# blackle/Megalania

Hardware: AMD Instinct MI355X
Metric: SA neighbour-cost evals/s (higher is better)
Workload: dtype u64

## Files before the change

### megalania_amd/csrc/mgl_api.hip

```cpp
#include "mgl_kernels.hip"
#include "mgl_kernels2.hip"
#include "mgl_kernels3.hip"
#include "mgl_kernels4.hip"
#include "mgl_kernels5.hip"
#include "mgl_pbuild.hip"
#include "mgl_index.hip"
#include "mgl_matchfinder.hip"
#include "mgl_optimal.hip"
#include "mgl_adaptive.hip"
#include "mgl_props.hip"
#include "mgl_crossover.hip"
#include "../../include/megalania_hip.h"

#include <math.h>
#include <stdio.h>
#include <stdlib.h>
#include <string.h>
#include <string>
#include <vector>

static const uint16_t k_cost_table[2048] = {
#include "mgl_cost_table.inc"
};

// ... 65 lines not shown
	uint16_t* d_cost_tbl;
	BaseMem base, scratch;
	mgl_pk* d_best;
	NbrOut nbr;
	uint32_t* d_aos;
	uint64_t* d_cum;
	uint16_t* d_final_probs;
	mgl_pk* d_topk_pk;
	uint64_t* d_topk_cost;
	uint32_t* d_small;
	uint32_t* d_sub_offs;
	uint32_t* d_sub_lens;
	uint32_t sub_cap;
	uint64_t sqrt_thresh;
	uint32_t per_wave_bytes, waves_per_block, nbr_lds, walk_lds;
	bool incremental;
	Base2 b2;
	unsigned long long* d_prof;
	uint32_t* d_todo;
	uint32_t per_wave2, waves_per_block2, nbr2_lds, build_lds;
	uint32_t big_waves = MGL_BIG_WAVES;
	uint32_t chg_cap = MGL_CHG_CAP;
	uint32_t per_wave_pick, per_wave_rest, pick_waves;
	size_t b2_bytes;
	BigScratch big;
	uint32_t* d_todo2;
	uint4* d_pickstate;
	uint4* d_pickrec;
	bool split_nbr, adaptive;
	bool form_single = false;
	uint32_t* d_counts;
	ApplyBuf ab;
	uint32_t apply_blocks;
	bool incremental_apply;
	bool snapshots;
	Base2 snap_lit, snap_best;
	SnapMeta* d_snap_meta;
	bool parallel_build;
	PBuild pb;
	hipEvent_t ev_begin, ev_end;
	std::vector<hipEvent_t> ev_pool;
	int accept_mode = MGL_ACCEPT_AUTO;
	uint32_t bulk_threshold = 0;
	bool bulk_now = true;
	uint64_t bulk_hold = 0;
	uint64_t blk_done = 0;
// ... 286 lines not shown
	}
	if (!sa->incremental) {
		const uint32_t blocks = (K + sa->waves_per_block - 1) / sa->waves_per_block;
		hipLaunchKernelGGL(k_neighbours, dim3(blocks), dim3(64 * sa->waves_per_block), sa->nbr_lds, sa->stream, sa->ctx, sa->base.v,
		                   (const Control*)sa->base.ctl, sa->cfg.seed, step_override, K, sa->nbr, sa->per_wave_bytes,
		                   (const uint32_t*)nullptr, (const uint32_t*)nullptr); NBR_TRACE("k_neighbours");
		HIPCHK(hipGetLastError());
		return MGL_OK;
	}
	if (zero_counts) HIPCHK(hipMemsetAsync(sa->d_counts, 0, 8 * sizeof(uint32_t), sa->stream));
	const uint32_t blocks2 = (K + sa->waves_per_block2 - 1) / sa->waves_per_block2;
	const bool split_now = sa->split_nbr && !sa->form_single;
	const uint32_t sim_lds_regular = ((((sa->ctx.L.total + 31u) >> 5) + 3u) & ~3u) * 4u + sa->chg_cap * 16u;
	if (split_now) {
		const uint32_t slices = nbr_slices(sa);
		HIPCHK(hipEventRecord(sa->ev_fork, sa->stream));
		if (slices >= 2) HIPCHK(hipStreamWaitEvent(sa->stream2, sa->ev_fork, 0));
#if !MGL_TAIL_EARLY
		HIPCHK(hipStreamWaitEvent(sa->stream3, sa->ev_fork, 0));
#endif
		for (uint32_t h = 0; h < slices; h++) {
			const uint32_t j0 = (uint32_t)((uint64_t)K * h / slices), j1 = (uint32_t)((uint64_t)K * (h + 1) / slices);
			hipStream_t st = (h & 1u) ? sa->stream2 : sa->stream;
			hipLaunchKernelGGL((sa->d_prof ? k_neighbours2<false, MGL_NBR_PICK, true> : k_neighbours2<false, MGL_NBR_PICK>), dim3((j1 - j0 + sa->pick_waves - 1) / sa->pick_waves), dim3(64 * sa->pick_waves),
			                   (MGL_PICK_T_GLOBAL ? 0u : 4096u) + sa->pick_waves * sa->per_wave_pick, st, sa->ctx,
			                   sa->b2, sa->base.ctl, sa->cfg.seed, step_override, K, sa->nbr, sa->per_wave_pick, sa->d_todo, sa->d_counts,
			                   sa->d_prof, sa->big, sa->d_pickrec, j0, j1, sa->d_pickstate); NBR_TRACE("k_neighbours2<false, MGL_NBR_PICK>");
			hipLaunchKernelGGL((k_neighbours2<false, MGL_NBR_REST>), dim3(j1 - j0), dim3(64), sa->per_wave_rest, st, sa->ctx,
			                   sa->b2, sa->base.ctl, sa->cfg.seed, step_override, K, sa->nbr, sa->per_wave_rest, sa->d_todo, sa->d_counts,
			                   g_prof_big ? (unsigned long long*)nullptr : sa->d_prof, sa->big, sa->d_pickrec, j0, j1, sa->d_pickstate); NBR_TRACE("k_neighbours2<false, MGL_NBR_REST>");
			HIPCHK(hipEventRecord(sa->ev_rest[h], st));
		}
		HIPCHK(hipGetLastError());
		for (uint32_t h = 0; h < slices; h++) {
			const uint32_t j0 = (uint32_t)((uint64_t)K * h / slices), j1 = (uint32_t)((uint64_t)K * (h + 1) / slices);
			HIPCHK(hipStreamWaitEvent(sa->stream3, sa->ev_rest[h], 0));
			if (sa->time_sim_step >= 0 && h < 2) HIPCHK(hipEventRecord(sim_event(sa, 4 * (size_t)sa->time_sim_step + 2 * h), sa->stream3));
			if (sa->count_traffic)
				hipLaunchKernelGGL(k_sim<true>, dim3(j1 - j0), dim3(64 * sa->sim_waves), sim_lds_regular, sa->stream3, sa->ctx, sa->b2, sa->base.ctl,
				                   sa->nbr, sa->big, j0, j1, sa->d_traffic);
			else
				hipLaunchKernelGGL(k_sim<false>, dim3(j1 - j0), dim3(64 * sa->sim_waves), sim_lds_regular, sa->stream3, sa->ctx, sa->b2, sa->base.ctl,
				                   sa->nbr, sa->big, j0, j1, (unsigned long long*)nullptr);
			NBR_TRACE("k_sim");
			if (sa->time_sim_step >= 0 && h < 2) HIPCHK(hipEventRecord(sim_event(sa, 4 * (size_t)sa->time_sim_step + 2 * h + 1), sa->stream3));
		}
// ... 416 lines not shown
			HIPCHK(hipMemset(sa->d_todo2, 0, sizeof(uint32_t) * (K + 1)));
		}
		{
			uint32_t best_w = 1, best_total = 0;
			for (uint32_t w = 1; w <= 8; w++) {
				const uint32_t bytes = 4096u + w * sa->per_wave2;
				if (bytes > 160u * 1024u) break;
				const uint32_t tot = (160u * 1024u / bytes) * w;
				if (tot > best_total) { best_total = tot; best_w = w; }
			}
			(void)best_w;
			sa->waves_per_block2 = 1;
		}
		sa->nbr2_lds = 4096u + sa->waves_per_block2 * sa->per_wave2;
		sa->build_lds = 4096u + ckpt_elems * 2u + ckpt_elems * 8u;
		HIPCHK(hipMalloc(&sa->d_counts, sizeof(uint32_t) * 16));
		HIPCHK(hipMemset(sa->d_counts, 0, sizeof(uint32_t) * 16));
		sa->big.todo_in = sa->d_todo; sa->big.todo_in_count = sa->d_counts; sa->big.spill_ctr = sa->d_counts + 2;
		HIPCHK(hipFuncSetAttribute((const void*)k_neighbours2<false, MGL_NBR_FULL>, hipFuncAttributeMaxDynamicSharedMemorySize, (int)sa->nbr2_lds));
		HIPCHK(hipFuncSetAttribute((const void*)k_neighbours2<false, MGL_NBR_PICK>, hipFuncAttributeMaxDynamicSharedMemorySize, 160 * 1024));
		HIPCHK(hipFuncSetAttribute((const void*)k_neighbours2<false, MGL_NBR_PICK, true>, hipFuncAttributeMaxDynamicSharedMemorySize, 160 * 1024));
		HIPCHK(hipFuncSetAttribute((const void*)k_neighbours2<false, MGL_NBR_REST>, hipFuncAttributeMaxDynamicSharedMemorySize, (int)sa->nbr2_lds));
		HIPCHK(hipFuncSetAttribute((const void*)k_neighbours2<true, MGL_NBR_FULL>, hipFuncAttributeMaxDynamicSharedMemorySize, (int)(4096u + sa->per_wave2 + 12u * MGL_BIG_CAP + MGL_COOP_BYTES)));
		HIPCHK(hipMalloc(&sa->d_pickrec, sizeof(uint4) * K));
		HIPCHK(hipMalloc(&sa->d_pickstate, sizeof(uint4) * 2 * K));
		sa->split_nbr = getenv("MGL_NO_SPLIT") == nullptr;
		if (sa->split_nbr) {
			BigScratch& g = sa->big;
			HIPCHK(hipMalloc(&g.sim_hdr, sizeof(uint4) * (size_t)K));
			HIPCHK(hipMalloc(&g.sim_keys, sizeof(uint16_t) * 2u * sa->chg_cap * (size_t)K));
			HIPCHK(hipMalloc(&g.sim_pos, sizeof(uint32_t) * 2u * sa->chg_cap * (size_t)K));
			HIPCHK(hipMemset(g.sim_hdr, 0xFF, sizeof(uint4) * (size_t)K));
			if (getenv("MGL_NO_CONT") == nullptr) {
				HIPCHK(hipMalloc(&g.cont, sizeof(uint32_t) * MGL_CONT_WORDS * (size_t)g.slots));
				HIPCHK(hipMemset(g.cont, 0, sizeof(uint32_t) * MGL_CONT_WORDS * (size_t)g.slots));
			}
		}
		if (getenv("MGL_SIMW")) { const int w = atoi(getenv("MGL_SIMW")); if (w == 1 || w == 2 || w == 4 || w == 8) sa->sim_waves = (uint32_t)w; }
		sa->adaptive = sa->split_nbr && getenv("MGL_NO_ADAPT") == nullptr;
		sa->form_single = !sa->split_nbr;
		sa->pick_waves = getenv("MGL_PICK_WAVES") ? (uint32_t)atoi(getenv("MGL_PICK_WAVES")) : 0u;
		if (sa->pick_waves != 1 && sa->pick_waves != 2 && sa->pick_waves != 4 && sa->pick_waves != 8) sa->pick_waves = 0;
		{
			uint32_t best_w = 1, best_resident = 0;
			for (uint32_t w = 1; w <= 8; w *= 2) {
				const uint32_t bytes = (MGL_PICK_T_GLOBAL ? 0u : 4096u) + w * sa->per_wave_pick;
// ... 1351 lines not shown
		HIPCHK(hipMemcpy(v + 8, sa->d_counts, sizeof(uint32_t) * 8, hipMemcpyDeviceToHost));
		memcpy(out, v, sizeof v);
		return MGL_OK;
	}
	case 14: src = sa->ab.hdr; sz = sa->ab.hdr ? sizeof(uint32_t) * 16 : 0; break;
	case 16: src = sa->base.ctl; sz = sizeof(Control); break;
	case 15: src = sa->d_pickrec; sz = sa->d_pickrec ? sizeof(uint4) * sa->cfg.neighbours_per_step : 0; break;
	case 18: src = sa->d_quad_pos; sz = sizeof(uint32_t) * (sa->n - 1); break;
	case 19: src = sa->d_quad_nx; sz = sizeof(uint16_t) * (sa->n - 1); break;
	case 12: src = sa->d_bucket_off; sz = sizeof(uint32_t) * 65537; break;
	case 13: src = sa->d_bucket_pos; sz = sizeof(uint32_t) * (sa->n - 1); break;
	case 30: case 31: case 32: case 33: case 34: case 35: src = sa->d_xpos[what - 30]; sz = sizeof(uint32_t) * (sa->n - 1); break;
	case 40: case 41: case 42: case 43: case 44: case 45: src = sa->d_xrank[what - 40]; sz = src ? sizeof(uint32_t) * (sa->n - 1) : 0; break;
	case 50: case 51: case 52: case 53: case 54: case 55: src = sa->d_xrun[what - 50]; sz = src ? sizeof(uint32_t) * (sa->n - 1) : 0; break;
	case 60: case 61: case 62: case 63: case 64: case 65: src = sa->d_xnxb[what - 60]; sz = sa->n - 1; break;
	case 70: src = sa->d_oct_pos; sz = sizeof(uint32_t) * (sa->n - 1); break;
	case 71: src = sa->d_oct_rank; sz = sizeof(uint32_t) * (sa->n - 1); break;
	case 72: src = sa->d_oct_run; sz = sizeof(uint32_t) * (sa->n - 1); break;
	case 73: src = sa->d_oct_nx8; sz = sizeof(uint64_t) * (sa->n - 1); break;
	case 74: src = sa->d_hex_pos; sz = sizeof(uint32_t) * (sa->n - 1); break;
	case 75: src = sa->d_hex_rank; sz = sizeof(uint32_t) * (sa->n - 1); break;
	case 76: src = sa->d_hex_run; sz = sizeof(uint32_t) * (sa->n - 1); break;
	case 77: src = sa->d_hex_nx8; sz = sizeof(uint64_t) * (sa->n - 1); break;
	case 22: src = sa->nbr.win2; sz = sizeof(uint32_t) * sa->cfg.neighbours_per_step; break;
	case 21: src = sa->nbr.win; sz = sizeof(uint32_t) * 2 * sa->cfg.neighbours_per_step; break;
	case 11: src = sa->pb.acc; sz = sa->pb.acc ? sizeof(unsigned long long) * 8 : 0; break;
	default: return fail(MGL_EINVAL, "mgl_debug_dump: unknown selector");
	}
	*bytes = sz;
	if (sz > cap_bytes) return fail(MGL_ERANGE, "mgl_debug_dump: buffer too small");
	HIPCHK(hipMemcpy(out, src, sz, hipMemcpyDeviceToHost));
	if (what == 84) HIPCHK(hipMemset(sa->lim.why, 0, sizeof(uint32_t)));
	return MGL_OK;
}

extern "C" int mgl_debug_set(mgl_sa* sa, uint32_t key, uint64_t value)
{
	if (sa && key == 5) {
		sa->force_batch_late = (uint32_t)(value >> 32);
		sa->force_batch_fail = (uint32_t)value;
		if (sa->force_batch_late && !sa->force_batch_fail) sa->force_batch_fail = 1;
		return MGL_OK;
	}
	if (sa && key == 6) {
		const uint32_t id = (uint32_t)(value & 0xFFu);
		const uint64_t v = value >> 8;
// ... 38 lines not shown
```

### megalania_amd/csrc/mgl_kernels2.hip

```cpp
#include "mgl_base2.h"


struct BitAcc {
	uint32_t word;
	uint64_t bits;
};
__device__ __forceinline__ void bitacc_move(BitAcc& a, uint64_t* arr, uint32_t new_word, uint32_t lane)
{
	if (new_word == a.word) return;
	if (lane == 0) arr[a.word] = a.bits;
	for (uint32_t z = a.word + 1 + lane; z < new_word; z += 64) arr[z] = 0;
	a.word = new_word; a.bits = 0;
}

__device__ void build_body(const DevCtx& c, const Base2& b, Control* ctl, int check_cost)
{
	extern __shared__ __attribute__((aligned(16))) unsigned char smem[];
	uint16_t* T = (uint16_t*)smem;
	uint16_t* probs = (uint16_t*)(smem + 4096);
	uint32_t* cnt = (uint32_t*)(smem + 4096 + (size_t)b.ck_elems * 2);
	uint32_t* off = cnt + b.ck_elems;
	const uint32_t lane = threadIdx.x;
	const uint32_t total = c.L.total;
	if (check_cost && !ctl->accepted_flag) return;
// ... 471 lines not shown
	if (c.L.lc > 0) {
		const uint32_t wprev = (uint32_t)__shfl((int)win.byte, (int)((p - 1u - win.base) & 63u), 64);
		prev_byte = p == 0 ? 0u : (p - 1u >= win.base ? wprev : (uint32_t)c.data[p - 1u]);
	}
	mgl_wstate sv = st;
	sv.pos = p;
	sv.ctx_state = lit_steps(st.ctx_state, i);
	mgl_plan pl;
	mgl_plan_packet(&c.L, &sv, MGL_LITERAL, 0, 1, byte, 0, prev_byte, &pl);
	if (__ballot(active && pl.nev != 9u)) return 0;
	if (active) {
		uint32_t ctx, bit;
		mgl_plan_event(&pl, slot, &ctx, &bit);
		const uint32_t at = n + i * 9u + slot;
		if (INS) { ch.ins_key[at] = (uint16_t)(ctx | (bit << 15)); ch.ins_pos[at] = p; }
		else { ch.rem_key[at] = (uint16_t)ctx; ch.rem_pos[at] = p; }
	}
	n += 9u * take;
	st.pos += take;
	st.ctx_state = lit_steps(st.ctx_state, take);
	return take;
}

__device__ void model_load(const DevCtx& c, const Base2& b, uint16_t* probs, const uint16_t* T, uint32_t y, uint32_t lane)
{
	const uint32_t ck = y >> MGL_CK2_SHIFT;
	const uint4* src = (const uint4*)(b.ck_probs + (size_t)ck * b.ck_elems);
	uint4* dst = (uint4*)probs;
	const uint32_t n16 = b.ck_elems / 8u;
	for (uint32_t base = 0; base < n16; base += 256u) {
		uint4 r[4];
#pragma unroll
		for (uint32_t u = 0; u < 4; u++) { const uint32_t i = base + u * 64u + lane; if (i < n16) r[u] = src[i]; }
#pragma unroll
		for (uint32_t u = 0; u < 4; u++) { const uint32_t i = base + u * 64u + lane; if (i < n16) dst[i] = r[u]; }
	}
	const uint32_t first = ck << MGL_CK2_SHIFT;
	const uint64_t bits = b.onwalk[first >> 6] & ((y & 63u) ? ((1ull << (y & 63u)) - 1ull) : 0ull) & (~0ull << (first & 63u));
	wave_sync();
	if (bits) {
		const uint32_t start = uni(((first >> 6) << 6) + ctz64(bits));
		Walk w;
		walk_reset(w);
		w.st = uni_state(base_state_at(b, start));
		while (w.st.pos < y) {
			walk_window(w, c, b.slab, lane);
			if (w.st.ctx_state < 7u) {
// ... 15 lines not shown
					mgl_wstate sv = w.st;
					sv.pos = p; sv.ctx_state = lit_steps(w.st.ctx_state, i);
					mgl_plan pl;
					mgl_plan_packet(&c.L, &sv, MGL_LITERAL, 0, 1, byte, 0, prev_byte, &pl);
					if (!__ballot(active && pl.nev != 9u)) {
						uint32_t ctx = 0, bit = 0;
						if (active) mgl_plan_event(&pl, slot, &ctx, &bit);
						for (uint32_t r = 0; r < take; r++) {
							if (active && i == r) probs[ctx] = (uint16_t)mgl_prob_update(probs[ctx], bit);
							wave_sync();
						}
						w.st.pos += take; w.st.ctx_state = lit_steps(w.st.ctx_state, take);
						w.packets += take;
						continue;
					}
				}
			}
			const mgl_pk pk = walk_slab_at(w, w.st.pos);
			walk_packet<true>(w, c, probs, T, mgl_pk_type(pk), mgl_pk_dist(pk), mgl_pk_len(pk), lane);
		}
		wave_sync();
	}
}

__device__ __forceinline__ void walk_from_state(Walk& w, const mgl_wstate& st)
{
	walk_reset(w);
	w.st = st;
}

struct BigScratch {
	uint16_t* ins_key; uint32_t* ins_pos; uint16_t* rem_key; uint32_t* rem_pos; uint16_t* uctx;
	uint32_t cap, uctx_cap, slots;
	const uint32_t* todo_in; const uint32_t* todo_in_count;
	uint32_t* spill_ctr;
	uint32_t chg_cap;
	uint4* sim_hdr;
	uint16_t* sim_keys;
	uint32_t* sim_pos;
	uint32_t* cont;
};
#define MGL_CONT_WORDS 368u
#define MGL_CONT_MAGIC 0x434F4E54u
#ifndef MGL_PICK_T_GLOBAL
#define MGL_PICK_T_GLOBAL 1
#endif
#ifndef MGL_REST_WAVES_PER_SIMD
#define MGL_REST_WAVES_PER_SIMD 4
#endif
#define MGL_NBR_FULL 0
#define MGL_NBR_PICK 1
#define MGL_NBR_REST 2
#ifndef MGL_BIG_WAVES
#define MGL_BIG_WAVES 4u
#endif
#define MGL_COOP_SIM 1u
#define MGL_COOP_EXIT 2u
#define MGL_COOP_BYTES 128u
struct CoopCmd {
	uint32_t gen;
	uint32_t op;
	uint32_t slot;
	uint32_t n_ins, n_rem, nu, limit;
	uint32_t overlay;
	unsigned long long sum[MGL_BIG_WAVES];
};
static_assert(sizeof(CoopCmd) <= MGL_COOP_BYTES, "CoopCmd outgrew its LDS");
__device__ __forceinline__ CoopCmd* coop_cmd(unsigned char* smem, uint32_t per_wave_bytes)
{
	return (CoopCmd*)(smem + 4096u + per_wave_bytes + 12u * MGL_BIG_CAP);
}
__device__ __forceinline__ void coop_share(const DevCtx& c, const Base2& b, const BigScratch& big, unsigned long long* dbg, unsigned char* smem,
                                           uint32_t per_wave_bytes, const uint16_t* T, CoopCmd* cmd, uint32_t lane, uint32_t wid)
{
	const uint32_t slot = uni(cmd->slot), overlay = uni(cmd->overlay);
// ... 28 lines not shown
		cmd->overlay = overlay ? (uint32_t)((unsigned char*)overlay - smem) : 0u;
		cmd->gen = cmd->gen + 1u;
	}
	__syncthreads();
	coop_share(c, b, big, dbg, smem, per_wave_bytes, T, cmd, lane, 0u);
	uint64_t d = 0;
	for (uint32_t w = 0; w < (blockDim.x >> 6); w++) d += cmd->sum[w];
	wave_sync();
	return (int64_t)d;
}
__device__ __forceinline__ void coop_helpers(const DevCtx& c, const Base2& b, const BigScratch& big, unsigned long long* dbg, unsigned char* smem,
                                             uint32_t per_wave_bytes, const uint16_t* T, uint32_t lane, uint32_t wid)
{
	CoopCmd* cmd = coop_cmd(smem, per_wave_bytes);
	uint32_t seen = 0;
	for (;;) {
		__syncthreads();
		const uint32_t gen = uni(cmd->gen);
		if (uni(cmd->op) == MGL_COOP_EXIT || gen == seen) return;
		seen = gen;
		coop_share(c, b, big, dbg, smem, per_wave_bytes, T, cmd, lane, wid);
	}
}
template <bool BIG, int MODE, bool PROF = false>
__device__ __forceinline__ void nbr2_one(const DevCtx& c, const Base2& b, Control* ctl, uint64_t seed,
                                         uint64_t step_override, uint32_t K, const NbrOut& out, uint32_t per_wave_bytes,
                                         uint32_t* todo, uint32_t* todo_count, unsigned long long* prof_acc,
                                         const BigScratch& big, uint4* pickrec, uint32_t j_base, uint32_t j_end, uint4* pickstate,
                                         unsigned char* smem, const uint16_t* T, uint32_t unit, uint32_t lane, uint32_t wid)
{
	uint32_t j = j_base + unit;
	uint32_t slot = 0;
	const unsigned long long t_begin = prof_acc ? __builtin_readcyclecounter() : 0ull;
	if (BIG) {
		slot = unit;
		const uint32_t nflag = *big.todo_in_count;
		if (slot >= nflag) return;
		j = uni(big.todo_in[slot]);
		if (lane == 0) atomicAdd((unsigned long long*)&ctl->big_nbrs, 1ull);
	}
	if (j >= K || (!BIG && j >= j_end)) return;
	unsigned char* mine = smem + ((MODE == MGL_NBR_REST || (MODE == MGL_NBR_PICK && MGL_PICK_T_GLOBAL)) ? 0u : 4096u) + (size_t)wid * per_wave_bytes;
	Journal jn;
	jn.old = (mgl_pk*)mine;
	jn.neu = jn.old + MGL_MAX_DIFFS;
	jn.pos = (uint32_t*)(jn.neu + MGL_MAX_DIFFS);
	jn.count = 0; jn.overflow = false;
	Changes ch;
	ch.nbitwords = (c.L.total + 31u) >> 5;
	ch.ctxbits = jn.pos + MGL_MAX_DIFFS;
	unsigned char* uni_base = MODE == MGL_NBR_PICK ? mine : (unsigned char*)(ch.ctxbits + ((ch.nbitwords + 3u) & ~3u));
	uint16_t* probs = (uint16_t*)uni_base;
	uint32_t* lencost = (uint32_t*)(uni_base + (size_t)b.ck_elems * 2);
// ... 6 lines not shown
	if (BIG) {
		if (slot >= big.slots) {
			if (lane == 0) { const uint32_t s2 = atomicAdd(todo_count, 1u); todo[s2] = j; }
			return;
		}
		ch.ins_key = big.ins_key + (size_t)slot * big.cap; ch.ins_pos = big.ins_pos + (size_t)slot * big.cap;
		ch.rem_key = big.rem_key + (size_t)slot * big.cap; ch.rem_pos = big.rem_pos + (size_t)slot * big.cap;
		ch.uctx = big.uctx + (size_t)slot * big.uctx_cap;
		ch.cap = big.cap; ch.uctx_cap = big.uctx_cap;
	}
	ch.n_ins = ch.n_rem = 0; ch.direct = 0; ch.overflow = false; ch.list_full = false;
	bool too_many = false;
	bool spilled = BIG;

	const uint64_t gstep = step_override != ~0ull ? step_override : ctl->gstep;
	NbrRng rng; rng.key = mgl_rng_key(seed, gstep, j); rng.n = 0;
	uint32_t* const crec = (BIG && big.cont != nullptr) ? big.cont + (size_t)slot * MGL_CONT_WORDS : nullptr;
	bool resumed = false;
	if (BIG && crec != nullptr) resumed = uni(crec[0]) == MGL_CONT_MAGIC && uni(crec[1]) == j;

	uint32_t target;
	mgl_wstate nb;
	if (MODE == MGL_NBR_REST && lane == 0) big.sim_hdr[j] = make_uint4(0xFFFFFFFFu, 0u, 0u, 0u);
	if (MODE == MGL_NBR_REST) {
		const uint4 s0 = pickstate[2u * j], s1 = pickstate[2u * j + 1u];
		target = s0.x; rng.n = s0.y;
		nb.pos = target; nb.ctx_state = s0.z;
		nb.dists[0] = s0.w; nb.dists[1] = s1.x; nb.dists[2] = s1.y; nb.dists[3] = s1.z;
	} else if (BIG && resumed) {
		target = uni(crec[2]);
		nb.pos = uni(crec[3]); nb.ctx_state = uni(crec[4]);
		nb.dists[0] = uni(crec[5]); nb.dists[1] = uni(crec[6]); nb.dists[2] = uni(crec[7]); nb.dists[3] = uni(crec[8]);
	} else if (c.strat_pre != nullptr) {
		target = uni(c.strat_tgt[j]);
		rng.n = 1;
		nb = uni_state(base_state_at(b, target));
		if (MODE == MGL_NBR_PICK && lane == 0) {
			pickstate[2u * j] = make_uint4(target, rng.n, nb.ctx_state, nb.dists[0]);
			pickstate[2u * j + 1u] = make_uint4(nb.dists[1], nb.dists[2], nb.dists[3], 0u);
		}
	} else {
		uint32_t mydraw = lane < 32 ? mgl_rng_draw(rng.key, lane) % c.n : 0;
		bool on = lane < 32 && ((b.onwalk[mydraw >> 6] >> (mydraw & 63u)) & 1ull);
		unsigned long long m = __ballot(on);
		if (m) {
			int f = __ffsll((long long)m) - 1;
			target = rdlane(mydraw, (uint32_t)f);
			rng.n = (uint32_t)f + 1;
		} else {
			rng.n = 32;
			uint32_t p = rdlane(mydraw, 31);
			uint32_t wd = p >> 6;
			uint64_t bits = b.onwalk[wd] & (~0ull << (p & 63u));
			while (!bits && ++wd < b.nw0) bits = b.onwalk[wd];
			target = uni(bits ? (wd << 6) + ctz64(bits) : 0u);
		}
		nb = uni_state(base_state_at(b, target));
		if (MODE == MGL_NBR_PICK && lane == 0) {
			pickstate[2u * j] = make_uint4(target, rng.n, nb.ctx_state, nb.dists[0]);
			pickstate[2u * j + 1u] = make_uint4(nb.dists[1], nb.dists[2], nb.dists[3], 0u);
		}
	}
	Prof prof;
	prof_start(prof, MODE == MGL_NBR_PICK ? nullptr : prof_acc);
	ch.dbg = MODE == MGL_NBR_PICK ? nullptr : prof_acc;
	PickProf pp;
	pp.acc = PROF ? prof_acc + 32u + K : nullptr;
	pp.t = t_begin;
	ch.diag = c.diag_stop;
	const uint32_t pos = target;
	mgl_wstate bs = nb;
	Win win; win.base = 0xFFFFFFFFu; win.pk = 0; win.byte = 0;
	Walk tw;

	win_cover(win, c, b.slab, pos, lane);
	const mgl_pk first = win_pk(win, pos);
	mgl_pk m_first = first, m_second = 0;
	bool second_set = false, mutated = false;
	prof_mark(prof, 0, lane);
	if (c.diag_stop == 1) { if (lane == 0) { out.cost[j] = MGL_INVALID_COST; out.ndiffs[j] = 0; out.walked[j] = first; } return; }
	if (!(BIG && resumed) && pos + 1 < c.n && (nbr_draw(rng) % 2u) == 0) {
		const mgl_pk second = uni64(b.slab[pos + 1]);
		const uint32_t ft = mgl_pk_type(first), flen = mgl_pk_len(first);
		const uint32_t st = mgl_pk_type(second), slen = mgl_pk_len(second), sdist = mgl_pk_dist(second);
		if ((ft == MGL_LONG_REP || ft == MGL_MATCH) && flen > 2) {
			m_second = mgl_pack(ft, mgl_pk_dist(first), flen - 1);
			m_first = MGL_PK_LITERAL;
			if (MODE != MGL_NBR_PICK) { journal_set(jn, pos, first, m_first, lane); journal_set(jn, pos + 1, second, m_second, lane); }
			second_set = true; mutated = true;
		} else if ((ft == MGL_LITERAL || ft == MGL_SHORT_REP) && (st == MGL_MATCH || st == MGL_LONG_REP)) {
			uint32_t rep_start = pos - (st == MGL_LONG_REP ? mgl_dist_at(&nb, sdist) : sdist);
			if (slen < MGL_MAX_MATCH && rep_start > 0 && rep_start <= pos && win_byte(win, pos) == c.data[rep_start - 1]) {
				m_first = mgl_pack(st, sdist, slen + 1);
				if (MODE != MGL_NBR_PICK) journal_set(jn, pos, first, m_first, lane);
				mutated = true;
			}
		}
	}
	enum { P_MODEL, P_SIM, P_TOPK, P_WALK, P_OUT };
	uint32_t phase = mutated ? P_WALK : P_MODEL;
	if (MODE == MGL_NBR_PICK && mutated) return;
	TopkPlan plan;
	if (MODE == MGL_NBR_PICK) {
		if (PROF) pick_prof_mark(&pp, 0, lane);
		if (MGL_PICK_BATCH) topk_plan_make(plan, c, nb, lane);
		if (PROF) pick_prof_mark(&pp, 1, lane);
	}
	if (MODE == MGL_NBR_REST && c.diag_stop != 0 && c.diag_stop != 4 && c.diag_stop < 40) return;
	bool pick_is_mutation = !mutated;
	uint32_t pick_pos = pos;
	mgl_pk pick_inc = first;
	bool pick_best = false;
	bool have_pick = false;
	mgl_pk picked_pk = 0, resume_old = 0;
	uint32_t sim_limit = MGL_POS_INF;
	bool sim_overlay = false;
	int64_t delta = 0;
	bool generate_failed = false, sim_deferred = false, walk_long = false;
	uint32_t npicks = 0;
	uint32_t count = 0;
	uint32_t walked = 0;
	uint32_t wend = 0;
	uint32_t wsoft = 0xFFFFFFFFu, taint = 0xFu, dep = 0u;
// ... 2 lines not shown
	if (BIG && resumed) {
		bs.pos = uni(crec[9]); bs.ctx_state = uni(crec[10]);
		bs.dists[0] = uni(crec[11]); bs.dists[1] = uni(crec[12]); bs.dists[2] = uni(crec[13]); bs.dists[3] = uni(crec[14]);
		count = uni(crec[15]); walked = uni(crec[16]); npicks = uni(crec[17]); wsoft = uni(crec[18]); taint = uni(crec[19]); dep = uni(crec[20]);
		rng.n = uni(crec[21]); guard = uni(crec[22]); jn.count = uni(crec[23]); ch.n_ins = uni(crec[24]); ch.n_rem = uni(crec[25]);
		const uint32_t fl = uni(crec[26]);
		pick_best = (fl & 1u) != 0; second_set = (fl & 2u) != 0;
		pick_inc = (mgl_pk)uni(crec[28]) | ((mgl_pk)uni(crec[29]) << 32);
		resume_old = (mgl_pk)uni(crec[30]) | ((mgl_pk)uni(crec[31]) << 32);
		m_second = (mgl_pk)uni(crec[32]) | ((mgl_pk)uni(crec[33]) << 32);
		ch.direct = (int64_t)((uint64_t)uni(crec[34]) | ((uint64_t)uni(crec[35]) << 32));
		if (lane < jn.count) {
			jn.pos[lane] = crec[48u + lane];
			jn.old[lane] = reinterpret_cast<const mgl_pk*>(crec + 112u)[lane];
			jn.neu[lane] = reinterpret_cast<const mgl_pk*>(crec + 240u)[lane];
		}
		wave_sync();
		if (lane == 0) crec[0] = 0u;
		pick_pos = nb.pos;
		mutated = true; pick_is_mutation = false; first_packet = false;
		phase = P_MODEL;
	}
	if ((MODE == MGL_NBR_REST || (BIG && pickrec != nullptr)) && !mutated) {
		const uint4 rec = pickrec[j];
		if (!(rec.w & 1u)) { generate_failed = true; phase = P_OUT; }
		else {
			m_first = (mgl_pk)rec.x | ((mgl_pk)rec.y << 32);
			journal_set(jn, pos, first, m_first, lane);
			rng.n = rec.z;
			pick_is_mutation = false;
			phase = P_WALK;
		}
	}

	for (;;) {
		if (MODE == MGL_NBR_REST && (phase == P_MODEL || phase == P_TOPK)) { ch.overflow = true; phase = P_OUT; continue; }
		if (MODE != MGL_NBR_REST && phase == P_MODEL) {
			if ((ch.n_ins + ch.n_rem) != 0 && !spilled) {
				uint32_t sl = 0;
				if (lane == 0) sl = atomicAdd(big.spill_ctr, 1u);
				sl = uni(sl);
				if (sl >= big.slots) { ch.overflow = true; phase = P_OUT; continue; }
				uint16_t* gik = big.ins_key + (size_t)sl * big.cap; uint32_t* gip = big.ins_pos + (size_t)sl * big.cap;
				uint16_t* grk = big.rem_key + (size_t)sl * big.cap; uint32_t* grp = big.rem_pos + (size_t)sl * big.cap;
				for (uint32_t i = lane; i < ch.n_ins; i += 64) { gik[i] = ch.ins_key[i]; gip[i] = ch.ins_pos[i]; }
				for (uint32_t i = lane; i < ch.n_rem; i += 64) { grk[i] = ch.rem_key[i]; grp[i] = ch.rem_pos[i]; }
				__threadfence_block();
				wave_sync();
				ch.ins_key = gik; ch.ins_pos = gip; ch.rem_key = grk; ch.rem_pos = grp;
				ch.uctx = big.uctx + (size_t)sl * big.uctx_cap;
				ch.cap = big.cap; ch.uctx_cap = big.uctx_cap;
				spilled = true;
			}
			model_load(c, b, probs, T, pick_pos, lane);
			if (PROF) pick_prof_mark(&pp, 2, lane);
			if (!pick_is_mutation) prof_mark(prof, 5, lane);
			if (pick_is_mutation) {
				prof_mark(prof, 1, lane);
				if (c.diag_stop == 2) { if (lane == 0) { out.cost[j] = MGL_INVALID_COST; out.ndiffs[j] = 0; out.walked[j] = probs[lane]; } return; }
			}
			if ((ch.n_ins + ch.n_rem) != 0) { sim_limit = pick_pos; sim_overlay = true; phase = P_SIM; }
			else phase = P_TOPK;
		}
		if (MODE == MGL_NBR_REST && phase == P_SIM) {
			uint16_t* gk = big.sim_keys + (size_t)j * (2u * big.chg_cap);
			uint32_t* gp = big.sim_pos + (size_t)j * (2u * big.chg_cap);
			for (uint32_t e = lane; e < ch.n_ins; e += 64) { gk[e] = ch.ins_key[e]; gp[e] = ch.ins_pos[e]; }
			for (uint32_t e = lane; e < ch.n_rem; e += 64) { gk[big.chg_cap + e] = ch.rem_key[e]; gp[big.chg_cap + e] = ch.rem_pos[e]; }
			if (lane == 0) big.sim_hdr[j] = make_uint4(ch.n_ins, ch.n_rem, (uint32_t)(uint64_t)ch.direct, (uint32_t)((uint64_t)ch.direct >> 32));
			sim_deferred = true;
			phase = P_OUT;
			continue;
		}
		if (MODE == MGL_NBR_FULL && phase == P_SIM) {
			int64_t r;
			if (BIG) r = coop_sim(c, b, big, prof_acc, smem, per_wave_bytes, T, ch, slot, sim_limit, sim_overlay ? probs : nullptr, lane, &too_many);
			else r = chain_sim(b, ch, T, sim_limit, sim_overlay ? probs : nullptr, lane, &too_many);
			wave_sync();
			if (too_many) { phase = P_OUT; continue; }
			if (sim_overlay) { prof_mark(prof, 6, lane); phase = P_TOPK; }
			else { delta = r; prof_mark(prof, 4, lane); phase = P_OUT; }
		}
		if (MODE != MGL_NBR_REST && phase == P_TOPK) {
			walk_from_state(tw, nb);
			walk_window(tw, c, b.slab, lane);
			mgl_pk picked;
			bool ok;
			if constexpr (MODE == MGL_NBR_PICK) ok = pick_from_top_k<4, MGL_PICK_BATCH != 0, PROF>(c, tw, probs, T, lencost, pick_inc, pick_best, rng, lane, &picked, &plan, &pp);
			else ok = pick_from_top_k<1>(c, tw, probs, T, lencost, pick_inc, pick_best, rng, lane, &picked);
			if (MODE == MGL_NBR_PICK) {
				if (lane == 0) pickrec[j] = make_uint4((uint32_t)picked, (uint32_t)(picked >> 32), rng.n, ok ? 1u : 0u);
				if (PROF) pick_prof_mark(&pp, 14, lane);
				if (PROF && pp.acc && lane == 0) pp.acc[2u * MGL_PICK_STAGES + j] = __builtin_readcyclecounter() - t_begin;
				return;
			}
			if (pick_is_mutation) {
				if (!ok) { generate_failed = true; phase = P_OUT; continue; }
				m_first = picked;
				journal_set(jn, pos, first, m_first, lane);
				pick_is_mutation = false;
				prof_mark(prof, 2, lane);
				if (c.diag_stop == 3 || (c.diag_stop >= 31 && c.diag_stop <= 39)) { if (lane == 0) { out.cost[j] = MGL_INVALID_COST; out.ndiffs[j] = 0; out.walked[j] = (uint32_t)m_first; } return; }
			} else {
				picked_pk = ok ? picked : pick_inc;
				have_pick = true;
				prof_mark(prof, 7, lane);
			}
			win.base = 0xFFFFFFFFu;
			phase = P_WALK;
		}
		if (MODE != MGL_NBR_PICK && phase == P_WALK) {
			bool request_pick = false;
			while (nb.pos < c.n || bs.pos < c.n) {
				if (ch.overflow || jn.overflow || too_many || ++guard > (BIG ? (1u << 20) : 4096u)) { ch.overflow = true; break; }
// ... 178 lines not shown
			if (BIG) atomicAdd((unsigned long long*)&ctl->fallback_nbrs, 1ull);
			out.cost[j] = MGL_INVALID_COST; out.ndiffs[j] = 0; out.walked[j] = 0; out.win[2u * j] = pos; out.win[2u * j + 1u] = MGL_WIN_NONE;
		}
		return;
	}
	const uint64_t total = (uint64_t)((int64_t)ctl->rebuild_cost + delta + ch.direct);
	uint32_t nd = 0;
	for (uint32_t i = 0; i < jn.count; i++) {
		if (jn.old[i] == jn.neu[i]) continue;
		if (lane == 0) {
			out.dpos[(size_t)j * MGL_MAX_DIFFS + nd] = jn.pos[i];
			out.dold[(size_t)j * MGL_MAX_DIFFS + nd] = jn.old[i];
			out.dnew[(size_t)j * MGL_MAX_DIFFS + nd] = jn.neu[i];
		}
		nd++;
	}
	if (lane == 0) { if (!sim_deferred) out.cost[j] = total; out.ndiffs[j] = nd; out.walked[j] = walked; out.win[2u * j] = pos; out.win[2u * j + 1u] = wend; out.win2[j] = (wsoft < wend ? wsoft : wend) | (dep << 31); }
	if (prof_acc && lane == 0)
		prof_acc[32 + j] = ((__builtin_readcyclecounter() - t_begin) & 0xFFFFFFFFFFull) |
		                   ((unsigned long long)((ch.n_ins + ch.n_rem) & 0xFFFu) << 40) | ((unsigned long long)(walked & 0xFFFu) << 52);
}

template <bool BIG, int MODE, bool PROF = false>
__global__ void __launch_bounds__((MODE == MGL_NBR_PICK ? 512 : (BIG ? 64 * MGL_BIG_WAVES : 64)), (MODE == MGL_NBR_FULL ? (BIG ? 1 : MGL_NBR_WAVES_PER_SIMD) : (MODE == MGL_NBR_REST ? MGL_REST_WAVES_PER_SIMD : 4))) k_neighbours2(DevCtx c, Base2 b, Control* ctl, uint64_t seed,
                                                     uint64_t step_override, uint32_t K, NbrOut out, uint32_t per_wave_bytes,
                                                     uint32_t* todo, uint32_t* todo_count, unsigned long long* prof_acc,
                                                     BigScratch big, uint4* pickrec, uint32_t j_base, uint32_t j_end, uint4* pickstate)
{
	const uint32_t waves = blockDim.x >> 6;
	if (BIG && blockIdx.x >= *big.todo_in_count) return;
	extern __shared__ __attribute__((aligned(16))) unsigned char smem[];
	uint16_t* T = (uint16_t*)smem;
	if (BIG && threadIdx.x == 0) { CoopCmd* cmd = coop_cmd(smem, per_wave_bytes); cmd->gen = 0; cmd->op = MGL_COOP_SIM; }
	if (MODE == MGL_NBR_PICK && MGL_PICK_T_GLOBAL) {
		T = const_cast<uint16_t*>(c.cost_tbl);
	} else if (MODE != MGL_NBR_REST) {
		for (uint32_t i = threadIdx.x; i < 256; i += blockDim.x) reinterpret_cast<uint4*>(T)[i] = reinterpret_cast<const uint4*>(c.cost_tbl)[i];
		__syncthreads();
	}
	const uint32_t lane = threadIdx.x & 63u, wid = threadIdx.x >> 6;
	if (BIG) {
		if (wid != 0) { coop_helpers(c, b, big, prof_acc, smem, per_wave_bytes, T, lane, wid); return; }
		const uint32_t n = *big.todo_in_count;
		for (uint32_t unit = blockIdx.x; unit < n; unit += gridDim.x)
			nbr2_one<BIG, MODE, PROF>(c, b, ctl, seed, step_override, K, out, per_wave_bytes, todo, todo_count, prof_acc, big, pickrec, j_base, j_end, pickstate, smem, T, unit, lane, 0u);
		if (lane == 0) { CoopCmd* cmd = coop_cmd(smem, per_wave_bytes); cmd->op = MGL_COOP_EXIT; cmd->gen = cmd->gen + 1u; }
		__syncthreads();
	} else {
		nbr2_one<BIG, MODE, PROF>(c, b, ctl, seed, step_override, K, out, per_wave_bytes, todo, todo_count, prof_acc, big, pickrec, j_base, j_end, pickstate, smem, T,
		                    blockIdx.x * waves + wid, lane, wid);
	}
}


#ifndef MGL_SIM_WAVES
#define MGL_SIM_WAVES 2u
#endif
#define MGL_SIM_WAVES_MAX 8u
struct SimShared {
	uint16_t* T;
	uint32_t* dyn;
	unsigned long long* sum;
	uint32_t* nu_many;
};
// ... 113 lines not shown
```

Baseline: 14.94 million.

## Fuse pick and rest neighbour kernels into one per-wave launch

Adds a PICKWALK mode that runs the pick and rest halves of neighbour generation back to back in one single-wave block. The pick state is handed over in registers instead of being written to and re-read from global pickstate/pickrec buffers. This removes a kernel launch per slice and the global round trip, and skips re-reading the first token window. In exchange the pick stage loses its multi-wave blocks and occupancy bound, LDS is sized to the larger of the two halves, and the larger fused body may raise register pressure. The fused path is on by default and can be disabled with an environment variable.

```diff
diff --git a/megalania_amd/csrc/mgl_api.hip b/megalania_amd/csrc/mgl_api.hip
--- a/megalania_amd/csrc/mgl_api.hip
+++ b/megalania_amd/csrc/mgl_api.hip
@@ -111,6 +111,8 @@
 	uint32_t big_waves = MGL_BIG_WAVES;
 	uint32_t chg_cap = MGL_CHG_CAP;
 	uint32_t per_wave_pick, per_wave_rest, pick_waves;
+	bool fuse;
+	uint32_t fused_lds;
 	size_t b2_bytes;
 	BigScratch big;
 	uint32_t* d_todo2;
@@ -443,6 +445,13 @@
 		for (uint32_t h = 0; h < slices; h++) {
 			const uint32_t j0 = (uint32_t)((uint64_t)K * h / slices), j1 = (uint32_t)((uint64_t)K * (h + 1) / slices);
 			hipStream_t st = (h & 1u) ? sa->stream2 : sa->stream;
+			if (sa->fuse && !sa->d_prof) {
+				hipLaunchKernelGGL((k_neighbours2<false, MGL_NBR_PICKWALK>), dim3(j1 - j0), dim3(64), sa->fused_lds, st, sa->ctx,
+				                   sa->b2, sa->base.ctl, sa->cfg.seed, step_override, K, sa->nbr, sa->fused_lds, sa->d_todo, sa->d_counts,
+				                   (unsigned long long*)nullptr, sa->big, sa->d_pickrec, j0, j1, sa->d_pickstate); NBR_TRACE("k_neighbours2<false, MGL_NBR_PICKWALK>");
+				HIPCHK(hipEventRecord(sa->ev_rest[h], st));
+				continue;
+			}
 			hipLaunchKernelGGL((sa->d_prof ? k_neighbours2<false, MGL_NBR_PICK, true> : k_neighbours2<false, MGL_NBR_PICK>), dim3((j1 - j0 + sa->pick_waves - 1) / sa->pick_waves), dim3(64 * sa->pick_waves),
 			                   (MGL_PICK_T_GLOBAL ? 0u : 4096u) + sa->pick_waves * sa->per_wave_pick, st, sa->ctx,
 			                   sa->b2, sa->base.ctl, sa->cfg.seed, step_override, K, sa->nbr, sa->per_wave_pick, sa->d_todo, sa->d_counts,
@@ -905,6 +914,9 @@
 		HIPCHK(hipFuncSetAttribute((const void*)k_neighbours2<false, MGL_NBR_PICK, true>, hipFuncAttributeMaxDynamicSharedMemorySize, 160 * 1024));
 		HIPCHK(hipFuncSetAttribute((const void*)k_neighbours2<false, MGL_NBR_REST>, hipFuncAttributeMaxDynamicSharedMemorySize, (int)sa->nbr2_lds));
 		HIPCHK(hipFuncSetAttribute((const void*)k_neighbours2<true, MGL_NBR_FULL>, hipFuncAttributeMaxDynamicSharedMemorySize, (int)(4096u + sa->per_wave2 + 12u * MGL_BIG_CAP + MGL_COOP_BYTES)));
+		sa->fuse = getenv("MGL_NO_FUSE") == nullptr;
+		sa->fused_lds = (MGL_PICK_T_GLOBAL ? 0u : 4096u) + (sa->per_wave_pick > sa->per_wave_rest ? sa->per_wave_pick : sa->per_wave_rest);
+		HIPCHK(hipFuncSetAttribute((const void*)k_neighbours2<false, MGL_NBR_PICKWALK>, hipFuncAttributeMaxDynamicSharedMemorySize, (int)sa->fused_lds));
 		HIPCHK(hipMalloc(&sa->d_pickrec, sizeof(uint4) * K));
 		HIPCHK(hipMalloc(&sa->d_pickstate, sizeof(uint4) * 2 * K));
 		sa->split_nbr = getenv("MGL_NO_SPLIT") == nullptr;
@@ -2302,6 +2314,9 @@
 	case 75: src = sa->d_hex_rank; sz = sizeof(uint32_t) * (sa->n - 1); break;
 	case 76: src = sa->d_hex_run; sz = sizeof(uint32_t) * (sa->n - 1); break;
 	case 77: src = sa->d_hex_nx8; sz = sizeof(uint64_t) * (sa->n - 1); break;
+	case 23: src = sa->nbr.cost; sz = sizeof(uint64_t) * sa->cfg.neighbours_per_step; break;
+	case 24: src = sa->nbr.ndiffs; sz = sizeof(uint32_t) * sa->cfg.neighbours_per_step; break;
+	case 25: src = sa->nbr.walked; sz = sizeof(uint32_t) * sa->cfg.neighbours_per_step; break;
 	case 22: src = sa->nbr.win2; sz = sizeof(uint32_t) * sa->cfg.neighbours_per_step; break;
 	case 21: src = sa->nbr.win; sz = sizeof(uint32_t) * 2 * sa->cfg.neighbours_per_step; break;
 	case 11: src = sa->pb.acc; sz = sa->pb.acc ? sizeof(unsigned long long) * 8 : 0; break;
diff --git a/megalania_amd/csrc/mgl_kernels2.hip b/megalania_amd/csrc/mgl_kernels2.hip
--- a/megalania_amd/csrc/mgl_kernels2.hip
+++ b/megalania_amd/csrc/mgl_kernels2.hip
@@ -517,7 +517,7 @@
 	return take;
 }
 
-__device__ void model_load(const DevCtx& c, const Base2& b, uint16_t* probs, const uint16_t* T, uint32_t y, uint32_t lane)
+__device__ __forceinline__ void model_load_inl(const DevCtx& c, const Base2& b, uint16_t* probs, const uint16_t* T, uint32_t y, uint32_t lane)
 {
 	const uint32_t ck = y >> MGL_CK2_SHIFT;
 	const uint4* src = (const uint4*)(b.ck_probs + (size_t)ck * b.ck_elems);
@@ -579,6 +579,10 @@
 		wave_sync();
 	}
 }
+__device__ void model_load(const DevCtx& c, const Base2& b, uint16_t* probs, const uint16_t* T, uint32_t y, uint32_t lane)
+{
+	model_load_inl(c, b, probs, T, y, lane);
+}
 
 __device__ __forceinline__ void walk_from_state(Walk& w, const mgl_wstate& st)
 {
@@ -608,6 +612,17 @@
 #define MGL_NBR_FULL 0
 #define MGL_NBR_PICK 1
 #define MGL_NBR_REST 2
+#define MGL_NBR_PICKWALK 3
+struct PickHand {
+	uint32_t target, rng_n;
+	uint32_t ctx_state, dists[4];
+	mgl_pk first, second;
+	mgl_pk m_first, m_second;
+	uint32_t flags;
+};
+#define MGL_HAND_MUTATED 1u
+#define MGL_HAND_SECOND 2u
+#define MGL_HAND_OK 4u
 #ifndef MGL_BIG_WAVES
 #define MGL_BIG_WAVES 4u
 #endif
@@ -682,13 +697,15 @@
 		coop_share(c, b, big, dbg, smem, per_wave_bytes, T, cmd, lane, wid);
 	}
 }
-template <bool BIG, int MODE, bool PROF = false>
+template <bool BIG, int MODE, bool PROF = false, bool FUSED = false>
 __device__ __forceinline__ void nbr2_one(const DevCtx& c, const Base2& b, Control* ctl, uint64_t seed,
                                          uint64_t step_override, uint32_t K, const NbrOut& out, uint32_t per_wave_bytes,
                                          uint32_t* todo, uint32_t* todo_count, unsigned long long* prof_acc,
                                          const BigScratch& big, uint4* pickrec, uint32_t j_base, uint32_t j_end, uint4* pickstate,
-                                         unsigned char* smem, const uint16_t* T, uint32_t unit, uint32_t lane, uint32_t wid)
-{
+                                         unsigned char* smem, const uint16_t* T, uint32_t unit, uint32_t lane, uint32_t wid,
+                                         PickHand* hand = nullptr)
+{
+	static_assert(!FUSED || (!BIG && !PROF && (MODE == MGL_NBR_PICK || MODE == MGL_NBR_REST)), "the fused instance is the two halves of the regular launch");
 	uint32_t j = j_base + unit;
 	uint32_t slot = 0;
 	const unsigned long long t_begin = prof_acc ? __builtin_readcyclecounter() : 0ull;
@@ -741,7 +758,11 @@
 	uint32_t target;
 	mgl_wstate nb;
 	if (MODE == MGL_NBR_REST && lane == 0) big.sim_hdr[j] = make_uint4(0xFFFFFFFFu, 0u, 0u, 0u);
-	if (MODE == MGL_NBR_REST) {
+	if (MODE == MGL_NBR_REST && FUSED) {
+		target = hand->target; rng.n = hand->rng_n;
+		nb.pos = target; nb.ctx_state = hand->ctx_state;
+		nb.dists[0] = hand->dists[0]; nb.dists[1] = hand->dists[1]; nb.dists[2] = hand->dists[2]; nb.dists[3] = hand->dists[3];
+	} else if (MODE == MGL_NBR_REST) {
 		const uint4 s0 = pickstate[2u * j], s1 = pickstate[2u * j + 1u];
 		target = s0.x; rng.n = s0.y;
 		nb.pos = target; nb.ctx_state = s0.z;
@@ -754,7 +775,7 @@
 		target = uni(c.strat_tgt[j]);
 		rng.n = 1;
 		nb = uni_state(base_state_at(b, target));
-		if (MODE == MGL_NBR_PICK && lane == 0) {
+		if (MODE == MGL_NBR_PICK && !FUSED && lane == 0) {
 			pickstate[2u * j] = make_uint4(target, rng.n, nb.ctx_state, nb.dists[0]);
 			pickstate[2u * j + 1u] = make_uint4(nb.dists[1], nb.dists[2], nb.dists[3], 0u);
 		}
@@ -775,10 +796,14 @@
 			target = uni(bits ? (wd << 6) + ctz64(bits) : 0u);
 		}
 		nb = uni_state(base_state_at(b, target));
-		if (MODE == MGL_NBR_PICK && lane == 0) {
+		if (MODE == MGL_NBR_PICK && !FUSED && lane == 0) {
 			pickstate[2u * j] = make_uint4(target, rng.n, nb.ctx_state, nb.dists[0]);
 			pickstate[2u * j + 1u] = make_uint4(nb.dists[1], nb.dists[2], nb.dists[3], 0u);
 		}
+	}
+	if (MODE == MGL_NBR_PICK && FUSED) {
+		hand->target = target; hand->ctx_state = nb.ctx_state;
+		hand->dists[0] = nb.dists[0]; hand->dists[1] = nb.dists[1]; hand->dists[2] = nb.dists[2]; hand->dists[3] = nb.dists[3];
 	}
 	Prof prof;
 	prof_start(prof, MODE == MGL_NBR_PICK ? nullptr : prof_acc);
@@ -792,19 +817,29 @@
 	Win win; win.base = 0xFFFFFFFFu; win.pk = 0; win.byte = 0;
 	Walk tw;
 
-	win_cover(win, c, b.slab, pos, lane);
-	const mgl_pk first = win_pk(win, pos);
+	mgl_pk first;
+	if (MODE == MGL_NBR_REST && FUSED) first = hand->first;
+	else { win_cover(win, c, b.slab, pos, lane); first = win_pk(win, pos); }
+	if (MODE == MGL_NBR_PICK && FUSED) hand->first = uni64(first);
 	mgl_pk m_first = first, m_second = 0;
 	bool second_set = false, mutated = false;
 	prof_mark(prof, 0, lane);
 	if (c.diag_stop == 1) { if (lane == 0) { out.cost[j] = MGL_INVALID_COST; out.ndiffs[j] = 0; out.walked[j] = first; } return; }
-	if (!(BIG && resumed) && pos + 1 < c.n && (nbr_draw(rng) % 2u) == 0) {
+	if (MODE == MGL_NBR_REST && FUSED) {
+		mutated = (hand->flags & MGL_HAND_MUTATED) != 0; second_set = (hand->flags & MGL_HAND_SECOND) != 0;
+		if (mutated) {
+			m_first = hand->m_first; m_second = hand->m_second;
+			journal_set(jn, pos, first, m_first, lane);
+			if (second_set) journal_set(jn, pos + 1, hand->second, m_second, lane);
+		}
+	} else if (!(BIG && resumed) && pos + 1 < c.n && (nbr_draw(rng) % 2u) == 0) {
 		const mgl_pk second = uni64(b.slab[pos + 1]);
 		const uint32_t ft = mgl_pk_type(first), flen = mgl_pk_len(first);
 		const uint32_t st = mgl_pk_type(second), slen = mgl_pk_len(second), sdist = mgl_pk_dist(second);
 		if ((ft == MGL_LONG_REP || ft == MGL_MATCH) && flen > 2) {
 			m_second = mgl_pack(ft, mgl_pk_dist(first), flen - 1);
 			m_first = MGL_PK_LITERAL;
+			if (MODE == MGL_NBR_PICK && FUSED) hand->second = uni64(second);
 			if (MODE != MGL_NBR_PICK) { journal_set(jn, pos, first, m_first, lane); journal_set(jn, pos + 1, second, m_second, lane); }
 			second_set = true; mutated = true;
 		} else if ((ft == MGL_LITERAL || ft == MGL_SHORT_REP) && (st == MGL_MATCH || st == MGL_LONG_REP)) {
@@ -818,6 +853,10 @@
 	}
 	enum { P_MODEL, P_SIM, P_TOPK, P_WALK, P_OUT };
 	uint32_t phase = mutated ? P_WALK : P_MODEL;
+	if (MODE == MGL_NBR_PICK && FUSED) {
+		hand->m_first = uni64(m_first); hand->m_second = uni64(m_second); hand->rng_n = uni(rng.n);
+		hand->flags = (mutated ? MGL_HAND_MUTATED : 0u) | (second_set ? MGL_HAND_SECOND : 0u);
+	}
 	if (MODE == MGL_NBR_PICK && mutated) return;
 	TopkPlan plan;
 	if (MODE == MGL_NBR_PICK) {
@@ -866,7 +905,8 @@
 		phase = P_MODEL;
 	}
 	if ((MODE == MGL_NBR_REST || (BIG && pickrec != nullptr)) && !mutated) {
-		const uint4 rec = pickrec[j];
+		const uint4 rec = (MODE == MGL_NBR_REST && FUSED) ? make_uint4((uint32_t)hand->m_first, (uint32_t)(hand->m_first >> 32), hand->rng_n, (hand->flags & MGL_HAND_OK) ? 1u : 0u)
+		                                                   : pickrec[j];
 		if (!(rec.w & 1u)) { generate_failed = true; phase = P_OUT; }
 		else {
 			m_first = (mgl_pk)rec.x | ((mgl_pk)rec.y << 32);
@@ -896,7 +936,8 @@
 				ch.cap = big.cap; ch.uctx_cap = big.uctx_cap;
 				spilled = true;
 			}
-			model_load(c, b, probs, T, pick_pos, lane);
+			if constexpr (FUSED) model_load_inl(c, b, probs, T, pick_pos, lane);
+			else model_load(c, b, probs, T, pick_pos, lane);
 			if (PROF) pick_prof_mark(&pp, 2, lane);
 			if (!pick_is_mutation) prof_mark(prof, 5, lane);
 			if (pick_is_mutation) {
@@ -934,6 +975,7 @@
 			else ok = pick_from_top_k<1>(c, tw, probs, T, lencost, pick_inc, pick_best, rng, lane, &picked);
 			if (MODE == MGL_NBR_PICK) {
 				if (lane == 0) pickrec[j] = make_uint4((uint32_t)picked, (uint32_t)(picked >> 32), rng.n, ok ? 1u : 0u);
+				if (FUSED) { hand->m_first = uni64(picked); hand->rng_n = uni(rng.n); if (ok) hand->flags |= MGL_HAND_OK; }
 				if (PROF) pick_prof_mark(&pp, 14, lane);
 				if (PROF && pp.acc && lane == 0) pp.acc[2u * MGL_PICK_STAGES + j] = __builtin_readcyclecounter() - t_begin;
 				return;
@@ -1158,7 +1200,7 @@
 }
 
 template <bool BIG, int MODE, bool PROF = false>
-__global__ void __launch_bounds__((MODE == MGL_NBR_PICK ? 512 : (BIG ? 64 * MGL_BIG_WAVES : 64)), (MODE == MGL_NBR_FULL ? (BIG ? 1 : MGL_NBR_WAVES_PER_SIMD) : (MODE == MGL_NBR_REST ? MGL_REST_WAVES_PER_SIMD : 4))) k_neighbours2(DevCtx c, Base2 b, Control* ctl, uint64_t seed,
+__global__ void __launch_bounds__((MODE == MGL_NBR_PICK ? 512 : (BIG ? 64 * MGL_BIG_WAVES : 64)), (MODE == MGL_NBR_FULL ? (BIG ? 1 : MGL_NBR_WAVES_PER_SIMD) : (MODE == MGL_NBR_REST ? MGL_REST_WAVES_PER_SIMD : 4)))  k_neighbours2(DevCtx c, Base2 b, Control* ctl, uint64_t seed,
                                                      uint64_t step_override, uint32_t K, NbrOut out, uint32_t per_wave_bytes,
                                                      uint32_t* todo, uint32_t* todo_count, unsigned long long* prof_acc,
                                                      BigScratch big, uint4* pickrec, uint32_t j_base, uint32_t j_end, uint4* pickstate)
@@ -1168,14 +1210,24 @@
 	extern __shared__ __attribute__((aligned(16))) unsigned char smem[];
 	uint16_t* T = (uint16_t*)smem;
 	if (BIG && threadIdx.x == 0) { CoopCmd* cmd = coop_cmd(smem, per_wave_bytes); cmd->gen = 0; cmd->op = MGL_COOP_SIM; }
-	if (MODE == MGL_NBR_PICK && MGL_PICK_T_GLOBAL) {
+	if ((MODE == MGL_NBR_PICK || MODE == MGL_NBR_PICKWALK) && MGL_PICK_T_GLOBAL) {
 		T = const_cast<uint16_t*>(c.cost_tbl);
 	} else if (MODE != MGL_NBR_REST) {
 		for (uint32_t i = threadIdx.x; i < 256; i += blockDim.x) reinterpret_cast<uint4*>(T)[i] = reinterpret_cast<const uint4*>(c.cost_tbl)[i];
 		__syncthreads();
 	}
 	const uint32_t lane = threadIdx.x & 63u, wid = threadIdx.x >> 6;
-	if (BIG) {
+	if constexpr (MODE == MGL_NBR_PICKWALK) {
+		static_assert(!BIG && !PROF, "the fused instance is a regular launch without stage marks");
+		PickHand hand;
+		hand.target = 0; hand.rng_n = 0; hand.ctx_state = 0; hand.dists[0] = hand.dists[1] = hand.dists[2] = hand.dists[3] = 0;
+		hand.first = hand.second = hand.m_first = hand.m_second = 0; hand.flags = 0;
+		nbr2_one<false, MGL_NBR_PICK, false, true>(c, b, ctl, seed, step_override, K, out, per_wave_bytes, todo, todo_count, nullptr, big, pickrec, j_base, j_end, pickstate, smem, T,
+		                                           blockIdx.x, lane, 0u, &hand);
+		wave_sync();
+		nbr2_one<false, MGL_NBR_REST, false, true>(c, b, ctl, seed, step_override, K, out, per_wave_bytes, todo, todo_count, nullptr, big, pickrec, j_base, j_end, pickstate, smem, T,
+		                                           blockIdx.x, lane, 0u, &hand);
+	} else if (BIG) {
 		if (wid != 0) { coop_helpers(c, b, big, prof_acc, smem, per_wave_bytes, T, lane, wid); return; }
 		const uint32_t n = *big.todo_in_count;
 		for (uint32_t unit = blockIdx.x; unit < n; unit += gridDim.x)
```

New measurement: 15.57 million, median of 6. 4.3% higher.
